# ChristodoulosPappas/IPLS-Java-API

Hardware: AMD Instinct MI355X
Metric: aggregated-gradient GB/s (device-resident), 32 peers×4M doubles/partition (higher is better)
Workload: dtype f64

## Files before the change

ipls-java-api_amd/csrc/ipls_kernels.hpp:

```cpp
#pragma once

#include <hip/hip_runtime.h>
#include <stdint.h>

#ifndef IPLS_ROT
#define IPLS_ROT 0
#endif
#ifndef IPLS_ROUND_PAIRS
#define IPLS_ROUND_PAIRS 1
#endif

namespace ipls {

typedef double d2 __attribute__((ext_vector_type(2)));
typedef unsigned long long u2 __attribute__((ext_vector_type(2)));
typedef unsigned u4w __attribute__((ext_vector_type(4)));

constexpr int kBlock = 256;

enum Start : int { kAccum = 0, kZero = 1, kFirst = 2 };

struct PartDesc {
  int64_t len;
  unsigned long long* dst;
  const unsigned long long* init;
  const unsigned long long* rep;
  unsigned long long* avg;
};

#define IPLS_GLOBAL __attribute__((address_space(1)))
typedef const IPLS_GLOBAL u2* gcu2;
typedef IPLS_GLOBAL u2* gu2;
typedef const IPLS_GLOBAL unsigned long long* gcu64;
typedef IPLS_GLOBAL unsigned long long* gu64;

__device__ __forceinline__ double be_to_f64(unsigned long long v) {
  return __builtin_bit_cast(double, __builtin_bswap64(v));
}
__device__ __forceinline__ unsigned long long f64_to_be(double v) {
  return __builtin_bswap64(__builtin_bit_cast(unsigned long long, v));
}

template <bool NT>
__device__ __forceinline__ u2 ld16(const unsigned long long* p) {
  if constexpr (NT) return __builtin_nontemporal_load((gcu2)p);
  else return *(gcu2)p;
}
__device__ __forceinline__ unsigned long long ld8(const unsigned long long* p) { return *(gcu64)p; }
__device__ __forceinline__ void st8(unsigned long long* p, unsigned long long v) { *(gu64)p = v; }

template <bool BE>
__device__ __forceinline__ d2 decode2(u2 raw) {
  if constexpr (BE) {
    const unsigned long long a = raw.x, b = raw.y;
    u2 s;
    s.x = __builtin_bswap64(a);
    s.y = __builtin_bswap64(b);
    return __builtin_bit_cast(d2, s);
  } else {
    return __builtin_bit_cast(d2, raw);
  }
}
template <bool BE>
__device__ __forceinline__ u2 encode2(d2 v) {
  u2 raw = __builtin_bit_cast(u2, v);
  if constexpr (BE) {
    const unsigned long long a = raw.x, b = raw.y;
    raw.x = __builtin_bswap64(a);
    raw.y = __builtin_bswap64(b);
  }
  return raw;
}
template <bool BE>
__device__ __forceinline__ double decode1(unsigned long long raw) {
  if constexpr (BE) return be_to_f64(raw);
  else return __builtin_bit_cast(double, raw);
}

__host__ __device__ constexpr int64_t grid_blocks(int map, int64_t tiles) {
  return map == 2 ? (tiles + 7) / 8 * 8 : tiles;
}

__device__ __forceinline__ void map_block(int map, int nblocks, int tiles_per_part, int n_parts, int& q, int& t) {
  int b = blockIdx.x;
  if (map == 3) {
    if (b < n_parts) {
      q = b;
      t = tiles_per_part - 1;
    } else {
      b -= n_parts;
      q = b / (tiles_per_part - 1);
      t = b - q * (tiles_per_part - 1);
    }
    return;
  }
  if (map == 2) {
    const int per = nblocks >> 3;
    b = (blockIdx.x & 7) * per + (blockIdx.x >> 3);
    if (b >= tiles_per_part * n_parts) { q = n_parts; t = 0; return; }
  }
  if (map == 1) {
    q = b % n_parts;
    t = b / n_parts;
  } else {
    q = b / tiles_per_part;
    t = b - q * tiles_per_part;
  }
}

template <bool BE_IN, bool BE_OUT, int START, int G, int R, bool NT, int MAP, int BS, bool FIN, int SEQF>
__device__ __forceinline__ void reduce_tiles(
    const unsigned long long* const* __restrict__ bufs, const PartDesc* __restrict__ parts,
    int k, int tiles_per_part, int n_parts, int secure, const double* __restrict__ cnts) {
  constexpr int kBlock = BS;
  constexpr int64_t kTile = (int64_t)kBlock * 2 * R;
  int q, t;
  map_block(MAP, gridDim.x, tiles_per_part, n_parts, q, t);
  if (q >= n_parts) return;
  const int64_t L = parts[q].len;
  const int64_t base = (int64_t)t * kTile;
  if (base >= L) return;
  unsigned long long* __restrict__ dst = parts[q].dst;
  const unsigned long long* const* __restrict__ pb = bufs + (size_t)q * k;
  const int tid = threadIdx.x;
  const int j0 = (START == kFirst) ? 1 : 0;
  static_assert(!(FIN && BE_OUT), "the fused round writes native Weights");
  const unsigned long long* __restrict__ init = FIN ? parts[q].init : dst;
  const unsigned long long* __restrict__ rep = FIN ? parts[q].rep : nullptr;
  unsigned long long* __restrict__ avg = FIN ? parts[q].avg : nullptr;
  double den = 0.0, cnt = 0.0;
  if constexpr (FIN) {
    if (avg) {
      cnt = cnts[q];
      den = secure ? 1e12 * cnt : cnt;
    }
  }
  const bool avg_aligned = FIN && !((uintptr_t)avg & 15);
  auto fin1 = [&](int64_t e, double a) {
    const double w = a + (rep ? __builtin_bit_cast(double, ld8(rep + e)) : 0.0);
    st8(dst + e, __builtin_bit_cast(unsigned long long, w));
    if (avg && e < L - 1) st8(avg + e, __builtin_bit_cast(unsigned long long, cnt == 0.0 ? w : w / den));
  };

  if (base + kTile <= L) {
    int64_t off[R];
#if IPLS_ROT
    const int rot = t & (R - 1);
#else
    constexpr int rot = 0;
#endif
    constexpr bool PAIRS = FIN && IPLS_ROUND_PAIRS && (R % 2 == 0);
    if constexpr (PAIRS) {
#pragma unroll
      for (int r = 0; r < R; ++r)
        off[r] = base + 2 * ((int64_t)(r >> 1) * 2 * kBlock + (tid >> 6) * 128 + (r & 1) * 64 + (tid & 63));
    } else {
#pragma unroll
      for (int r = 0; r < R; ++r) off[r] = base + 2 * ((int64_t)((r + rot) & (R - 1)) * kBlock + tid);
    }

    constexpr bool SEQ = SEQF > 0 && G == 1;
    d2 acc[R];
#pragma unroll
    for (int r = 0; r < R; ++r) {
      if constexpr (START == kZero) {
        acc[r] = d2{0.0, 0.0};
      } else if constexpr (START == kFirst) {
        acc[r] = decode2<BE_IN>(ld16<NT>(pb[0] + off[r]));
      } else {
        acc[r] = decode2<BE_OUT>(ld16<false>(init + off[r]));
      }
      if constexpr (SEQ && START != kZero) __builtin_amdgcn_sched_barrier(0);
    }
    int j = j0;
    if constexpr (SEQ) {
      for (; j < k; ++j) {
        const unsigned long long* __restrict__ src = pb[j];
#pragma unroll
        for (int r = 0; r < R; ++r) {
          const d2 x = decode2<BE_IN>(ld16<NT>(src + off[r]));
          acc[r].x = acc[r].x + x.x;
          acc[r].y = acc[r].y + x.y;
          if constexpr (SEQF > 0)
            if ((r + 1) % (SEQF % 10) == 0 && r + 1 < R - SEQF / 10) __builtin_amdgcn_sched_barrier(0);
        }
      }
    } else {
    for (; j + G <= k; j += G) {
      u2 v[G][R];
#pragma unroll
      for (int g = 0; g < G; ++g) {
        const unsigned long long* __restrict__ src = pb[j + g];
#pragma unroll
        for (int r = 0; r < R; ++r) v[g][r] = ld16<NT>(src + off[r]);
      }
#pragma unroll
      for (int g = 0; g < G; ++g) {
#pragma unroll
        for (int r = 0; r < R; ++r) {
          d2 x = decode2<BE_IN>(v[g][r]);
          acc[r].x = acc[r].x + x.x;
          acc[r].y = acc[r].y + x.y;
        }
      }
    }
    for (; j < k; ++j) {
      const unsigned long long* __restrict__ src = pb[j];
      u2 v[R];
#pragma unroll
      for (int r = 0; r < R; ++r) v[r] = ld16<NT>(src + off[r]);
#pragma unroll
      for (int r = 0; r < R; ++r) {
        d2 x = decode2<BE_IN>(v[r]);
        acc[r].x = acc[r].x + x.x;
        acc[r].y = acc[r].y + x.y;
      }
    }
    }
    if constexpr (FIN) {
#pragma unroll
      for (int r = 0; r < R; ++r) {
        if (rep) {
          const d2 y = decode2<false>(ld16<true>(rep + off[r]));
          acc[r].x = acc[r].x + y.x;
          acc[r].y = acc[r].y + y.y;
        } else {
          acc[r].x = acc[r].x + 0.0;
          acc[r].y = acc[r].y + 0.0;
        }
        if (avg) {
          const int64_t e = off[r];
          const double ax = cnt == 0.0 ? acc[r].x : acc[r].x / den;
          const double ay = cnt == 0.0 ? acc[r].y : acc[r].y / den;
          if (avg_aligned) {
            if (e + 1 < L - 1) __builtin_nontemporal_store(encode2<false>(d2{ax, ay}), (gu2)(avg + e));
            else st8(avg + e, __builtin_bit_cast(unsigned long long, ax));
          } else if constexpr (PAIRS) {
            const int lane = tid & 63;
            const double nx = __shfl_down(ax, 1);
            if ((r & 1) == 0) {
              const double nb = acc[r + 1].x + (rep && lane == 0 ? __builtin_bit_cast(double, ld8(rep + off[r + 1])) : 0.0);
              const double b0 = __shfl(cnt == 0.0 ? nb : nb / den, 0);
              if (lane == 0) st8(avg + e, __builtin_bit_cast(unsigned long long, ax));
              __builtin_nontemporal_store(encode2<false>(d2{ay, lane < 63 ? nx : b0}), (gu2)(avg + e + 1));
            } else {
              if (lane < 63) __builtin_nontemporal_store(encode2<false>(d2{ay, nx}), (gu2)(avg + e + 1));
              else if (e + 1 < L - 1) st8(avg + e + 1, __builtin_bit_cast(unsigned long long, ay));
            }
          } else {
            const double nx = __shfl_down(ax, 1);
            const int lane = tid & 63;
            if (lane == 0) st8(avg + e, __builtin_bit_cast(unsigned long long, ax));
            if (lane < 63) __builtin_nontemporal_store(encode2<false>(d2{ay, nx}), (gu2)(avg + e + 1));
            else if (e + 1 < L - 1) st8(avg + e + 1, __builtin_bit_cast(unsigned long long, ay));
          }
        }
      }
#pragma unroll
      for (int r = 0; r < R; ++r) __builtin_nontemporal_store(encode2<false>(acc[r]), (gu2)(dst + off[r]));
    } else {
#pragma unroll
      for (int r = 0; r < R; ++r) __builtin_nontemporal_store(encode2<BE_OUT>(acc[r]), (gu2)(dst + off[r]));
    }
  } else {
    constexpr int kPB = 8;
    for (int64_t sb = base; sb < L; sb += 2 * kBlock) {
      const int64_t i = sb + 2 * tid;
      if (sb + 2 * kBlock <= L) {
        d2 acc;
        if constexpr (START == kZero) acc = d2{0.0, 0.0};
        else if constexpr (START == kFirst) acc = decode2<BE_IN>(ld16<NT>(pb[0] + i));
        else acc = decode2<BE_OUT>(ld16<false>(init + i));
        int jj = j0;
        for (; jj + kPB <= k; jj += kPB) {
          u2 v[kPB];
#pragma unroll
          for (int g = 0; g < kPB; ++g) v[g] = ld16<NT>(pb[jj + g] + i);
#pragma unroll
          for (int g = 0; g < kPB; ++g) {
            const d2 x = decode2<BE_IN>(v[g]);
            acc.x = acc.x + x.x;
            acc.y = acc.y + x.y;
          }
        }
        for (; jj < k; ++jj) {
          const d2 x = decode2<BE_IN>(ld16<NT>(pb[jj] + i));
          acc.x = acc.x + x.x;
          acc.y = acc.y + x.y;
        }
        if constexpr (FIN) {
          fin1(i, acc.x);
          fin1(i + 1, acc.y);
        } else {
          __builtin_nontemporal_store(encode2<BE_OUT>(acc), (gu2)(dst + i));
        }
      } else {
        for (int64_t e = sb + tid; e < L; e += kBlock) {
          double acc;
          if constexpr (START == kZero) acc = 0.0;
          else if constexpr (START == kFirst) acc = decode1<BE_IN>(ld8(pb[0] + e));
          else acc = decode1<BE_OUT>(ld8(init + e));
          int jj = j0;
          for (; jj + kPB <= k; jj += kPB) {
            unsigned long long v[kPB];
#pragma unroll
            for (int g = 0; g < kPB; ++g) v[g] = ld8(pb[jj + g] + e);
#pragma unroll
            for (int g = 0; g < kPB; ++g) acc = acc + decode1<BE_IN>(v[g]);
          }
          for (; jj < k; ++jj) acc = acc + decode1<BE_IN>(ld8(pb[jj] + e));
          if constexpr (FIN) fin1(e, acc);
          else st8(dst + e, BE_OUT ? f64_to_be(acc) : __builtin_bit_cast(unsigned long long, acc));
        }
      }
    }
  }
}

template <bool BE_IN, bool BE_OUT, int START, int G, int R, bool NT, int MAP = 0, int BS = kBlock, int SEQF = 0>
__global__ __launch_bounds__(BS) void k_reduce(const unsigned long long* const* __restrict__ bufs,
                                               const PartDesc* __restrict__ parts, int k, int tiles_per_part,
                                               int n_parts) {
  reduce_tiles<BE_IN, BE_OUT, START, G, R, NT, MAP, BS, false, SEQF>(bufs, parts, k, tiles_per_part, n_parts, 0,
                                                                     nullptr);
}

template <bool BE_IN, int START, int G, int R, int MAP = 0, int BS = kBlock, int SEQF = 0>
__global__ __launch_bounds__(BS) void k_round(const unsigned long long* const* __restrict__ bufs,
                                              const PartDesc* __restrict__ parts, int k, int tiles_per_part,
                                              int n_parts, int secure, const double* __restrict__ cnts) {
  reduce_tiles<BE_IN, false, START, G, R, true, MAP, BS, true, SEQF>(bufs, parts, k, tiles_per_part, n_parts, secure,
                                                               cnts);
}

constexpr int kEwV = 4;
constexpr int64_t kEwTile = (int64_t)kBlock * 2 * kEwV;

template <bool BE_IN, bool FIRST, bool VEC = false>
__global__ __launch_bounds__(kBlock) void k_fold_n(unsigned long long* __restrict__ dst,
                                                   const unsigned long long* __restrict__ src, int64_t n) {
  auto one = [&](int64_t i) {
    const double x = decode1<BE_IN>(ld8(src + i));
    const double y = FIRST ? x : __builtin_bit_cast(double, ld8(dst + i)) + x;
    st8(dst + i, __builtin_bit_cast(unsigned long long, y));
  };
  if constexpr (VEC) {
    const int64_t base = (int64_t)blockIdx.x * kEwTile;
    if (base + kEwTile <= n) {
      u2 sv[kEwV], dv[kEwV];
#pragma unroll
      for (int v = 0; v < kEwV; ++v) {
        const int64_t i = base + 2 * ((int64_t)v * kBlock + threadIdx.x);
        sv[v] = __builtin_nontemporal_load((gcu2)(src + i));
        if constexpr (!FIRST) dv[v] = *(gcu2)(dst + i);
      }
#pragma unroll
      for (int v = 0; v < kEwV; ++v) {
        const int64_t i = base + 2 * ((int64_t)v * kBlock + threadIdx.x);
        d2 o = decode2<BE_IN>(sv[v]);
        if constexpr (!FIRST) {
          const d2 y = __builtin_bit_cast(d2, dv[v]);
          o.x = y.x + o.x;
          o.y = y.y + o.y;
        }
        *(gu2)(dst + i) = __builtin_bit_cast(u2, o);
      }
      return;
    }
    for (int64_t i = base + threadIdx.x; i < n; i += kBlock) one(i);
  } else {
    for (int64_t i = (int64_t)blockIdx.x * kBlock + threadIdx.x; i < n; i += (int64_t)gridDim.x * kBlock) one(i);
  }
}

template <bool BE_IN, int START>
__global__ __launch_bounds__(64) void k_round_counts(const unsigned long long* const* __restrict__ bufs,
                                                     const PartDesc* __restrict__ parts, int k, int n_parts,
                                                     double* __restrict__ cnts) {
  const int q = blockIdx.x;
  if (q >= n_parts) return;
  const int lane = threadIdx.x;
  const PartDesc d = parts[q];
  const int64_t e = d.len - 1;
  const unsigned long long* const* pb = bufs + (size_t)q * k;
  double c = (START == kZero) ? 0.0 : __builtin_bit_cast(double, ld8(d.init + e));
  for (int j0 = 0; j0 < k; j0 += 64) {
    const int j = j0 + lane;
    const double v = j < k ? decode1<BE_IN>(ld8(pb[j] + e)) : 0.0;
    const int m = k - j0 < 64 ? k - j0 : 64;
    for (int t = 0; t < m; ++t) c = c + __shfl(v, t);
  }
  if (lane == 0) cnts[q] = c + (d.rep ? __builtin_bit_cast(double, ld8(d.rep + e)) : 0.0);
}

template <bool BE_IN, bool BE_OUT, int START>
__global__ __launch_bounds__(kBlock) void k_reduce_scalar(
    const unsigned long long* const* __restrict__ bufs, const PartDesc* __restrict__ parts,
    int k, int tiles_per_part, int64_t tile) {
  const int q = blockIdx.x / tiles_per_part;
  const int t = blockIdx.x - q * tiles_per_part;
  const int64_t L = parts[q].len;
  const int64_t base = (int64_t)t * tile;
  if (base >= L) return;
  unsigned long long* __restrict__ dst = parts[q].dst;
  const unsigned long long* const* __restrict__ pb = bufs + (size_t)q * k;
  const int64_t end = (base + tile < L) ? base + tile : L;
  const int j0 = (START == kFirst) ? 1 : 0;
  for (int64_t i = base + threadIdx.x; i < end; i += kBlock) {
    double acc;
    if constexpr (START == kZero) acc = 0.0;
    else if constexpr (START == kFirst) acc = decode1<BE_IN>(ld8(pb[0] + i));
    else acc = decode1<BE_OUT>(ld8(dst + i));
    for (int j = j0; j < k; ++j) acc = acc + decode1<BE_IN>(ld8(pb[j] + i));
    st8(dst + i, BE_OUT ? f64_to_be(acc) : __builtin_bit_cast(unsigned long long, acc));
  }
}

template <bool BE_IN, bool BE_OUT, int START, int R = 4>
__global__ __launch_bounds__(kBlock) void k_fold1(unsigned long long* __restrict__ dst,
                                                  const unsigned long long* __restrict__ src, int64_t L) {
  const int64_t n2 = L >> 1;
  const int64_t stride = (int64_t)gridDim.x * kBlock * R;
  auto fold = [&](const u2& v, const u2& t) -> u2 {
    const d2 x = decode2<BE_IN>(v);
    if constexpr (START == kFirst) return encode2<BE_OUT>(x);
    d2 a = (START == kZero) ? d2{0.0, 0.0} : decode2<BE_OUT>(t);
    a.x = a.x + x.x;
    a.y = a.y + x.y;
    return encode2<BE_OUT>(a);
  };
  int64_t b = (int64_t)blockIdx.x * kBlock * R + threadIdx.x;
  for (; b + (int64_t)(R - 1) * kBlock < n2; b += stride) {
    u2 v[R], t[R];
#pragma unroll
    for (int r = 0; r < R; ++r) v[r] = ld16<true>(src + 2 * (b + r * kBlock));
    if constexpr (START == kAccum) {
#pragma unroll
      for (int r = 0; r < R; ++r) t[r] = ld16<false>(dst + 2 * (b + r * kBlock));
    }
#pragma unroll
    for (int r = 0; r < R; ++r) __builtin_nontemporal_store(fold(v[r], t[r]), (gu2)(dst + 2 * (b + r * kBlock)));
  }
  for (int r = 0; r < R; ++r) {
    const int64_t i2 = b + r * kBlock;
    if (i2 < n2) {
      const u2 t = (START == kAccum) ? ld16<false>(dst + 2 * i2) : u2{0, 0};
      __builtin_nontemporal_store(fold(ld16<true>(src + 2 * i2), t), (gu2)(dst + 2 * i2));
    }
  }
  if ((L & 1) && blockIdx.x == 0 && threadIdx.x == 0) {
    const int64_t e = L - 1;
    const double x = decode1<BE_IN>(ld8(src + e));
    double a;
    if constexpr (START == kFirst) a = x;
    else a = ((START == kZero) ? 0.0 : decode1<BE_OUT>(ld8(dst + e))) + x;
    st8(dst + e, BE_OUT ? f64_to_be(a) : __builtin_bit_cast(unsigned long long, a));
  }
}

struct FinDesc {
  int64_t len;
  int64_t agg_off, rep_off, w_off;
};

constexpr int kFinV = 8, kDivV = 4;
constexpr int64_t kFinTile = (int64_t)kBlock * 2 * kFinV, kDivTile = (int64_t)kBlock * 2 * kDivV;

template <bool REP_ZERO, bool ZERO_ACC, int BS = kBlock, int V = kFinV>
__global__ __launch_bounds__(BS) void k_finalize(const FinDesc* __restrict__ parts,
                                                 double* __restrict__ arena,
                                                 int tiles_per_part) {
  constexpr int kBlock = BS;
  constexpr int kV = V;
  constexpr int64_t kTile = (int64_t)kBlock * 2 * kV;
  const int q = blockIdx.x / tiles_per_part;
  const int t = blockIdx.x - q * tiles_per_part;
  const FinDesc d = parts[q];
  const int64_t base = (int64_t)t * kTile;
  if (base >= d.len) return;
  const int64_t end = (base + kTile < d.len) ? base + kTile : d.len;
  double* agg = arena + d.agg_off;
  double* rep = arena + d.rep_off;
  double* w = arena + d.w_off;
  if (end - base == kTile) {
    u2 a[kV], r[kV];
#pragma unroll
    for (int v = 0; v < kV; ++v) {
      const int64_t i = base + 2 * ((int64_t)v * kBlock + threadIdx.x);
      a[v] = __builtin_nontemporal_load((gcu2)(agg + i));
      if constexpr (!REP_ZERO) r[v] = __builtin_nontemporal_load((gcu2)(rep + i));
    }
#pragma unroll
    for (int v = 0; v < kV; ++v) {
      const int64_t i = base + 2 * ((int64_t)v * kBlock + threadIdx.x);
      const d2 x = __builtin_bit_cast(d2, a[v]);
      const d2 y = REP_ZERO ? d2{0.0, 0.0} : __builtin_bit_cast(d2, r[v]);
      d2 o;
      o.x = x.x + y.x;
      o.y = x.y + y.y;
      __builtin_nontemporal_store(__builtin_bit_cast(u2, o), (gu2)(w + i));
      if constexpr (ZERO_ACC) {
        __builtin_nontemporal_store(u2{0, 0}, (gu2)(agg + i));
        if constexpr (!REP_ZERO) __builtin_nontemporal_store(u2{0, 0}, (gu2)(rep + i));
      }
    }
    return;
  }
  for (int64_t i = base + threadIdx.x; i < end; i += kBlock) {
    const double a = agg[i];
    const double r = REP_ZERO ? 0.0 : rep[i];
    w[i] = a + r;
    if constexpr (ZERO_ACC) {
      agg[i] = 0.0;
      if constexpr (!REP_ZERO) rep[i] = 0.0;
    }
  }
}

struct DivDesc {
  int64_t len;
  int64_t w_off;
  int64_t out_off;
};

template <bool OUT_BE, bool SECURE, int BS = kBlock, int V = kDivV>
__global__ __launch_bounds__(BS) void k_divide(const DivDesc* __restrict__ parts,
                                               const double* __restrict__ arena,
                                               unsigned long long* __restrict__ out,
                                               int tiles_per_part) {
  constexpr int kBlock = BS;
  constexpr int kV = V;
  constexpr int64_t kTile = (int64_t)kBlock * 2 * kV;
  static_assert(BS % 64 == 0, "whole waves");
  const int q = blockIdx.x / tiles_per_part;
  const int t = blockIdx.x - q * tiles_per_part;
  const DivDesc d = parts[q];
  const int64_t n = d.len - 1;
  const double* w = arena + d.w_off;
  const double cnt = w[d.len - 1];
  const double den = SECURE ? 1e12 * cnt : cnt;
  auto f = [&](double x) -> unsigned long long {
    const double y = (cnt == 0.0) ? x : x / den;
    unsigned long long bits = __builtin_bit_cast(unsigned long long, y);
    if constexpr (OUT_BE) {
      if (y != y) bits = 0x7ff8000000000000ULL;
      bits = __builtin_bswap64(bits);
    }
    return bits;
  };
  unsigned long long* o = out + d.out_off;
  const int64_t to_line = (16 - (int64_t)(((uintptr_t)o >> 3) & 15)) & 15;
  const int64_t head = to_line < n ? to_line : n;
  if (t == 0 && threadIdx.x < head) o[threadIdx.x] = f(w[threadIdx.x]);
  const int64_t base = (int64_t)t * kTile + head;
  if (base >= n) return;
  if (base + kTile <= n) {
    const int64_t wave_base = base + (int64_t)(threadIdx.x >> 6) * 128 * kV + 2 * (threadIdx.x & 63);
    double x[kV][2];
#pragma unroll
    for (int v = 0; v < kV; ++v) {
      const int64_t i = wave_base + (int64_t)v * 128;
      x[v][0] = __builtin_nontemporal_load((const __attribute__((address_space(1))) double*)(w + i));
      x[v][1] = __builtin_nontemporal_load((const __attribute__((address_space(1))) double*)(w + i + 1));
    }
#pragma unroll
    for (int v = 0; v < kV; ++v) {
      const int64_t i = wave_base + (int64_t)v * 128;
      u2 v2;
      v2.x = f(x[v][0]);
      v2.y = f(x[v][1]);
      __builtin_nontemporal_store(v2, (gu2)(o + i));
    }
    return;
  }
  for (int64_t i = base + threadIdx.x; i < n; i += kBlock) o[i] = f(w[i]);
}

template <bool BE_IN, bool BE_OUT, int MODE, bool VEC = false>
__global__ __launch_bounds__(kBlock) void k_split(const unsigned long long* __restrict__ flat,
                                                  int64_t lo, int64_t ncopy, int64_t L,
                                                  unsigned long long* __restrict__ dst) {
  static_assert(MODE == 0 || !BE_OUT, "the folds write native doubles");
  auto one = [&](int64_t i) {
    double v;
    if (i < ncopy) v = decode1<BE_IN>(flat[lo + i]);
    else if (i == ncopy) v = 1.0;
    else v = 0.0;
    if constexpr (MODE == 1) {
      const double a = __builtin_bit_cast(double, dst[i]);
      dst[i] = __builtin_bit_cast(unsigned long long, a + v);
    } else if constexpr (MODE == 2) {
      dst[i] = __builtin_bit_cast(unsigned long long, 0.0 + v);
    } else {
      dst[i] = BE_OUT ? f64_to_be(v) : __builtin_bit_cast(unsigned long long, v);
    }
  };
  if constexpr (VEC) {
    const int64_t base = (int64_t)blockIdx.x * kEwTile;
    if (base + kEwTile <= ncopy) {
      const unsigned long long* src = flat + lo;
      u2 sv[kEwV], dv[kEwV];
#pragma unroll
      for (int k = 0; k < kEwV; ++k) {
        const int64_t i = base + 2 * ((int64_t)k * kBlock + threadIdx.x);
        sv[k] = __builtin_nontemporal_load((gcu2)(src + i));
        if constexpr (MODE == 1) dv[k] = *(gcu2)(dst + i);
      }
#pragma unroll
      for (int k = 0; k < kEwV; ++k) {
        const int64_t i = base + 2 * ((int64_t)k * kBlock + threadIdx.x);
        const d2 x = decode2<BE_IN>(sv[k]);
        d2 o;
        if constexpr (MODE == 1) {
          const d2 a = __builtin_bit_cast(d2, dv[k]);
          o = d2{a.x + x.x, a.y + x.y};
        } else if constexpr (MODE == 2) {
          o = d2{0.0 + x.x, 0.0 + x.y};
        } else {
          o = x;
        }
        *(gu2)(dst + i) = encode2<BE_OUT>(o);
      }
      return;
    }
    const int64_t end = base + kEwTile < L ? base + kEwTile : L;
    for (int64_t i = base + threadIdx.x; i < end; i += kBlock) one(i);
  } else {
    const int64_t i = (int64_t)blockIdx.x * kBlock + threadIdx.x;
    if (i < L) one(i);
  }
}

template <bool VEC = false>
__global__ __launch_bounds__(kBlock) void k_bswap64(const unsigned long long* __restrict__ in,
                                                    unsigned long long* __restrict__ out, int64_t n) {
  if constexpr (VEC) {
    const int64_t base = (int64_t)blockIdx.x * kEwTile;
    if (base + kEwTile <= n) {
      u2 v[kEwV];
#pragma unroll
      for (int k = 0; k < kEwV; ++k) v[k] = __builtin_nontemporal_load((gcu2)(in + base + 2 * ((int64_t)k * kBlock + threadIdx.x)));
#pragma unroll
      for (int k = 0; k < kEwV; ++k) {
        const unsigned long long a = v[k].x, b = v[k].y;
        __builtin_nontemporal_store(u2{__builtin_bswap64(a), __builtin_bswap64(b)},
                                    (gu2)(out + base + 2 * ((int64_t)k * kBlock + threadIdx.x)));
      }
      return;
    }
    for (int64_t i = base + threadIdx.x; i < n; i += kBlock) out[i] = __builtin_bswap64(in[i]);
  } else {
    for (int64_t i = (int64_t)blockIdx.x * kBlock + threadIdx.x; i < n; i += (int64_t)gridDim.x * kBlock)
      out[i] = __builtin_bswap64(in[i]);
  }
}

template <bool BE_IN>
__global__ __launch_bounds__(kBlock) void k_load_model(const unsigned long long* __restrict__ flat,
                                                       int64_t lo, int64_t ncopy, int64_t L,
                                                       double* __restrict__ dst) {
  const int64_t i = (int64_t)blockIdx.x * kBlock + threadIdx.x;
  if (i >= L) return;
  dst[i] = (i < ncopy) ? decode1<BE_IN>(flat[lo + i]) : 0.0;
}

__device__ __forceinline__ unsigned long long splitmix64(unsigned long long v) {
  unsigned long long z = v + 0x9E3779B97F4A7C15ULL;
  z = (z ^ (z >> 30)) * 0xBF58476D1CE4E5B9ULL;
  z = (z ^ (z >> 27)) * 0x94D049BB133111EBULL;
  return z ^ (z >> 31);
}

template <bool BE_OUT>
__global__ __launch_bounds__(kBlock) void k_synth(unsigned long long* __restrict__ dst, int64_t L,
                                                  unsigned long long key) {
  for (int64_t i = (int64_t)blockIdx.x * kBlock + threadIdx.x; i < L;
       i += (int64_t)gridDim.x * kBlock) {
    double x;
    if (i == L - 1) {
      x = 1.0;
    } else {
      const double u = (double)(splitmix64(key ^ (unsigned long long)i) >> 11) * 0x1.0p-53;
      double tt = 2.0 * u;
      tt = tt - 1.0;
      x = tt * 1e-2;
    }
    dst[i] = BE_OUT ? f64_to_be(x) : __builtin_bit_cast(unsigned long long, x);
  }
}

__device__ __forceinline__ unsigned long long dpp_shift(unsigned long long v, int ctrl_id) {
  const int lo = (int)(unsigned)v, hi = (int)(unsigned)(v >> 32);
  int rl, rh;
  switch (ctrl_id) {
    case 0: rl = __builtin_amdgcn_update_dpp(0, lo, 0x111, 0xF, 0xF, true);
            rh = __builtin_amdgcn_update_dpp(0, hi, 0x111, 0xF, 0xF, true); break;
    case 1: rl = __builtin_amdgcn_update_dpp(0, lo, 0x112, 0xF, 0xF, true);
            rh = __builtin_amdgcn_update_dpp(0, hi, 0x112, 0xF, 0xF, true); break;
    case 2: rl = __builtin_amdgcn_update_dpp(0, lo, 0x114, 0xF, 0xF, true);
            rh = __builtin_amdgcn_update_dpp(0, hi, 0x114, 0xF, 0xF, true); break;
    case 3: rl = __builtin_amdgcn_update_dpp(0, lo, 0x118, 0xF, 0xF, true);
            rh = __builtin_amdgcn_update_dpp(0, hi, 0x118, 0xF, 0xF, true); break;
    case 4: rl = __builtin_amdgcn_update_dpp(0, lo, 0x142, 0xA, 0xF, false);
            rh = __builtin_amdgcn_update_dpp(0, hi, 0x142, 0xA, 0xF, false); break;
    default: rl = __builtin_amdgcn_update_dpp(0, lo, 0x143, 0xC, 0xF, false);
             rh = __builtin_amdgcn_update_dpp(0, hi, 0x143, 0xC, 0xF, false); break;
  }
  return ((unsigned long long)(unsigned)rh << 32) | (unsigned)rl;
}

__device__ __forceinline__ unsigned long long wave_sum_u64(unsigned long long v) {
#pragma unroll
  for (int c = 0; c < 6; ++c) v += dpp_shift(v, c);
  const unsigned lo = __builtin_amdgcn_readlane((int)(unsigned)v, 63);
  const unsigned hi = __builtin_amdgcn_readlane((int)(unsigned)(v >> 32), 63);
  return ((unsigned long long)hi << 32) | lo;
}

template <bool BE_IN>
__global__ __launch_bounds__(kBlock) void k_checksum(const unsigned long long* __restrict__ x,
                                                     int64_t n, unsigned long long* __restrict__ out) {
  __shared__ unsigned long long lds[kBlock / 64];
  unsigned long long s = 0;
  for (int64_t i = (int64_t)blockIdx.x * kBlock + threadIdx.x; i < n;
       i += (int64_t)gridDim.x * kBlock) {
    unsigned long long b = BE_IN ? __builtin_bswap64(x[i]) : x[i];
    s += splitmix64(b + (unsigned long long)i * 0x9E3779B97F4A7C15ULL);
  }
  s = wave_sum_u64(s);
  const int lane = threadIdx.x & 63, wid = threadIdx.x >> 6;
  if (lane == 0) lds[wid] = s;
  __syncthreads();
  if (threadIdx.x == 0) {
    unsigned long long t = 0;
#pragma unroll
    for (int w = 0; w < kBlock / 64; ++w) t += lds[w];
    atomicAdd(out, t);
  }
}

struct B64Desc {
  int64_t src_off;
  int64_t units;
  int64_t dst_off;
  int32_t tail;
  int32_t pad;
};

__device__ __forceinline__ unsigned b64url_val(unsigned c) {
  if (c - 'A' < 26u) return c - 'A';
  if (c - 'a' < 26u) return c - 'a' + 26;
  if (c - '0' < 10u) return c - '0' + 52;
  if (c == '-') return 62;
  if (c == '_') return 63;
  return 0x100;
}

__device__ __forceinline__ unsigned b64url_unit(unsigned w) {
  const unsigned a = b64url_val(w & 0xFF), b = b64url_val((w >> 8) & 0xFF);
  const unsigned c = b64url_val((w >> 16) & 0xFF), d = b64url_val(w >> 24);
  return (a << 18) | (b << 12) | (c << 6) | d | ((a | b | c | d) & 0x100 ? 0x1000000u : 0u);
}

__global__ __launch_bounds__(kBlock) void k_b64url_decode(const unsigned char* __restrict__ src,
                                                          const B64Desc* __restrict__ descs,
                                                          unsigned char* __restrict__ dst,
                                                          int* __restrict__ err) {
  const int m = blockIdx.y;
  const B64Desc d = descs[m];
  const unsigned char* s = src + d.src_off;
  unsigned char* o = dst + d.dst_off;
  const int64_t u0 = ((int64_t)blockIdx.x * kBlock + threadIdx.x) * 4;
  if (u0 > d.units) return;
  unsigned bad = 0;
  if (u0 + 4 <= d.units) {
    typedef unsigned u4 __attribute__((ext_vector_type(4)));
    const u4 w = *(const IPLS_GLOBAL u4*)(s + 4 * u0);
    const unsigned v[4] = {b64url_unit(w.x), b64url_unit(w.y), b64url_unit(w.z), b64url_unit(w.w)};
    bad = (v[0] | v[1] | v[2] | v[3]) & 0x1000000u;
    unsigned char* q = o + 3 * u0;
#pragma unroll
    for (int i = 0; i < 4; ++i) {
      q[3 * i] = (unsigned char)(v[i] >> 16);
      q[3 * i + 1] = (unsigned char)(v[i] >> 8);
      q[3 * i + 2] = (unsigned char)v[i];
    }
  } else {
    for (int64_t u = u0; u < d.units; ++u) {
      const unsigned char* c = s + 4 * u;
      const unsigned w = c[0] | (c[1] << 8) | (c[2] << 16) | ((unsigned)c[3] << 24);
      const unsigned v = b64url_unit(w);
      bad |= v & 0x1000000u;
      o[3 * u] = (unsigned char)(v >> 16);
      o[3 * u + 1] = (unsigned char)(v >> 8);
      o[3 * u + 2] = (unsigned char)v;
    }
    if (d.tail && u0 + 4 > d.units) {
      const unsigned char* c = s + 4 * d.units;
      unsigned v = 0, inval = 0;
      for (int i = 0; i < d.tail; ++i) {
        const unsigned x = b64url_val(c[i]);
        inval |= x;
        v |= (x & 63u) << (18 - 6 * i);
      }
      bad |= inval & 0x100;
      o[3 * d.units] = (unsigned char)(v >> 16);
      if (d.tail == 3) o[3 * d.units + 1] = (unsigned char)(v >> 8);
    }
  }
  if (bad) atomicOr(err + m, 1);
}

struct FrameEnc {
  unsigned char hdr[16];
  int64_t n;
  int64_t origin_len;
  const unsigned char* origin;
};

__device__ __forceinline__ unsigned b64url_char(unsigned v) {
  return v < 26 ? 'A' + v : v < 52 ? 'a' + (v - 26) : v < 62 ? '0' + (v - 52) : v == 62 ? '-' : '_';
}
__device__ __forceinline__ unsigned b64url_quad(unsigned v) {
  return b64url_char((v >> 18) & 63) | (b64url_char((v >> 12) & 63) << 8) | (b64url_char((v >> 6) & 63) << 16) |
         (b64url_char(v & 63) << 24);
}

__device__ __forceinline__ unsigned frame_byte(const FrameEnc& f, const unsigned long long* __restrict__ src,
                                               int64_t j) {
  if (j < 14) return f.hdr[j];
  const int64_t q = j - 14;
  if (q < 8 * f.n) {
    if (!src) return 0;
    const unsigned long long v = ld8(src + (q >> 3));
    return (unsigned)(v >> (8 * (7 - (q & 7)))) & 0xFF;
  }
  return f.origin[q - 8 * f.n];
}

__device__ __forceinline__ unsigned b64url_quad_lut(const unsigned char* tab, unsigned v) {
  return (unsigned)tab[(v >> 18) & 63] | ((unsigned)tab[(v >> 12) & 63] << 8) | ((unsigned)tab[(v >> 6) & 63] << 16) |
         ((unsigned)tab[v & 63] << 24);
}

__device__ __forceinline__ void encode_frame_job(const FrameEnc& f, const unsigned long long* __restrict__ src,
                                                 unsigned char* __restrict__ out, int64_t groups, int64_t text_len,
                                                 const unsigned char* tab, u4w* stage) {
  const int lane = threadIdx.x & 63, wv = threadIdx.x >> 6;
  u4w* ws = stage + 128 * wv;
  const int64_t F = 14 + 8 * f.n + f.origin_len;
  for (int64_t g0 = (int64_t)blockIdx.x * kBlock; g0 < groups; g0 += (int64_t)gridDim.x * kBlock) {
    const int64_t gw = g0 + 64 * wv;
    const int64_t g = gw + lane;
    const int64_t b0 = 24 * g;
    u4w c0 = {0u, 0u, 0u, 0u}, c1 = {0u, 0u, 0u, 0u};
    if (g < groups && g >= 1 && b0 + 24 <= 14 + 8 * f.n && src) {
      const unsigned long long* s = src + (3 * g - 2);
      const unsigned long long v0 = ld8(s), v1 = ld8(s + 1), v2 = ld8(s + 2), v3 = ld8(s + 3);
      const unsigned W[8] = {(unsigned)(v0 >> 32), (unsigned)v0, (unsigned)(v1 >> 32), (unsigned)v1,
                             (unsigned)(v2 >> 32), (unsigned)v2, (unsigned)(v3 >> 32), (unsigned)v3};
      unsigned O[6];
#pragma unroll
      for (int k = 0; k < 6; ++k) O[k] = (W[k] << 16) | (W[k + 1] >> 16);
      const unsigned long long X0 = ((unsigned long long)O[0] << 32) | O[1];
      const unsigned long long X1 = ((unsigned long long)O[2] << 32) | O[3];
      const unsigned long long X2 = ((unsigned long long)O[4] << 32) | O[5];
      c0.x = b64url_quad_lut(tab, (unsigned)(X0 >> 40) & 0xFFFFFF);
      c0.y = b64url_quad_lut(tab, (unsigned)(X0 >> 16) & 0xFFFFFF);
      c0.z = b64url_quad_lut(tab, (unsigned)((X0 << 8) | (X1 >> 56)) & 0xFFFFFF);
      c0.w = b64url_quad_lut(tab, (unsigned)(X1 >> 32) & 0xFFFFFF);
      c1.x = b64url_quad_lut(tab, (unsigned)(X1 >> 8) & 0xFFFFFF);
      c1.y = b64url_quad_lut(tab, (unsigned)((X1 << 16) | (X2 >> 48)) & 0xFFFFFF);
      c1.z = b64url_quad_lut(tab, (unsigned)(X2 >> 24) & 0xFFFFFF);
      c1.w = b64url_quad_lut(tab, (unsigned)X2 & 0xFFFFFF);
    } else if (g < groups) {
      unsigned q8[8] = {0u, 0u, 0u, 0u, 0u, 0u, 0u, 0u};
      for (int u = 0; u < 8; ++u) {
        const int64_t j = b0 + 3 * u;
        if (j >= F) break;
        const int nb = F - j >= 3 ? 3 : (int)(F - j);
        unsigned v = frame_byte(f, src, j) << 16;
        if (nb > 1) v |= frame_byte(f, src, j + 1) << 8;
        if (nb > 2) v |= frame_byte(f, src, j + 2);
        unsigned q = b64url_quad(v);
        if (nb < 3) q = (q & 0x00FFFFFFu) | ((unsigned)'=' << 24);
        if (nb < 2) q = (q & 0xFF00FFFFu) | ((unsigned)'=' << 16);
        q8[u] = q;
      }
      c0 = u4w{q8[0], q8[1], q8[2], q8[3]};
      c1 = u4w{q8[4], q8[5], q8[6], q8[7]};
    }
    ws[2 * lane] = c0;
    ws[2 * lane + 1] = c1;
    __builtin_amdgcn_wave_barrier();
    const int64_t wbase = 32 * gw;
#pragma unroll
    for (int h = 0; h < 2; ++h) {
      const u4w v = ws[64 * h + lane];
      const int64_t o = wbase + 1024 * h + 16 * lane;
      if (o + 16 <= text_len) {
        __builtin_nontemporal_store(v, (IPLS_GLOBAL u4w*)(out + o));
      } else if (o < text_len) {
        const unsigned w4[4] = {v.x, v.y, v.z, v.w};
        for (int64_t c = 0; o + c < text_len; ++c) out[o + c] = (unsigned char)(w4[c >> 2] >> (8 * (c & 3)));
      }
    }
    __builtin_amdgcn_wave_barrier();
  }
}

__device__ __forceinline__ void init_b64url_table(unsigned char* tab) {
  if (threadIdx.x < 64) tab[threadIdx.x] = (unsigned char)b64url_char(threadIdx.x);
  __syncthreads();
}

__global__ __launch_bounds__(kBlock) void k_b64url_encode_frame(FrameEnc f, const unsigned long long* __restrict__ src,
                                                               unsigned char* __restrict__ out, int64_t groups,
                                                               int64_t text_len) {
  __shared__ u4w stage[2 * kBlock];
  __shared__ unsigned char tab[64];
  init_b64url_table(tab);
  encode_frame_job(f, src, out, groups, text_len, tab, stage);
}

struct FrameJob {
  FrameEnc f;
  const unsigned long long* src;
  unsigned char* out;
  int64_t groups;
  int64_t text_len;
};

__global__ __launch_bounds__(kBlock) void k_b64url_encode_frames(const FrameJob* __restrict__ jobs) {
  __shared__ u4w stage[2 * kBlock];
  __shared__ unsigned char tab[64];
  init_b64url_table(tab);
  const FrameJob& j = jobs[blockIdx.y];
  encode_frame_job(j.f, j.src, j.out, j.groups, j.text_len, tab, stage);
}

template <bool BE_IN, bool VEC = false>
__global__ __launch_bounds__(kBlock) void k_blend(double* __restrict__ t, const unsigned long long* __restrict__ g,
                                                  int64_t L, double a, double b) {
  auto one = [&](int64_t i) {
    const double x = decode1<BE_IN>(ld8(g + i));
    const double aw = a * t[i];
    const double bg = b * x;
    t[i] = aw + bg;
  };
  if constexpr (VEC) {
    const int64_t base = (int64_t)blockIdx.x * kEwTile;
    if (base + kEwTile <= L) {
      u2 gv[kEwV], tv[kEwV];
#pragma unroll
      for (int v = 0; v < kEwV; ++v) {
        const int64_t i = base + 2 * ((int64_t)v * kBlock + threadIdx.x);
        gv[v] = __builtin_nontemporal_load((gcu2)(g + i));
        tv[v] = *(gcu2)(t + i);
      }
#pragma unroll
      for (int v = 0; v < kEwV; ++v) {
        const int64_t i = base + 2 * ((int64_t)v * kBlock + threadIdx.x);
        const d2 x = decode2<BE_IN>(gv[v]);
        const d2 w = __builtin_bit_cast(d2, tv[v]);
        const double awx = a * w.x, bgx = b * x.x, awy = a * w.y, bgy = b * x.y;
        *(gu2)(t + i) = __builtin_bit_cast(u2, d2{awx + bgx, awy + bgy});
      }
      return;
    }
    for (int64_t i = base + threadIdx.x; i < L; i += kBlock) one(i);
  } else {
    for (int64_t i = (int64_t)blockIdx.x * kBlock + threadIdx.x; i < L; i += (int64_t)gridDim.x * kBlock) one(i);
  }
}

template <bool VEC = false>
__global__ __launch_bounds__(kBlock) void k_scale(double* __restrict__ d, const double* __restrict__ s, int64_t L,
                                                  double c) {
  if constexpr (VEC) {
    const int64_t base = (int64_t)blockIdx.x * kEwTile;
    if (base + kEwTile <= L) {
      u2 sv[kEwV];
#pragma unroll
      for (int v = 0; v < kEwV; ++v)
        sv[v] = __builtin_nontemporal_load((gcu2)(s + base + 2 * ((int64_t)v * kBlock + threadIdx.x)));
#pragma unroll
      for (int v = 0; v < kEwV; ++v) {
        const d2 x = __builtin_bit_cast(d2, sv[v]);
        __builtin_nontemporal_store(__builtin_bit_cast(u2, d2{c * x.x, c * x.y}),
                                    (gu2)(d + base + 2 * ((int64_t)v * kBlock + threadIdx.x)));
      }
      return;
    }
    for (int64_t i = base + threadIdx.x; i < L; i += kBlock) d[i] = c * s[i];
  } else {
    for (int64_t i = (int64_t)blockIdx.x * kBlock + threadIdx.x; i < L; i += (int64_t)gridDim.x * kBlock)
      d[i] = c * s[i];
  }
}

__device__ __forceinline__ double encode_secure1(double x) {
  if (x > 10.0) return 10 * 1e12;
  if (x < -10.0) return -10 * 1e12;
  return x * 1e12;
}

template <bool BE_IN, bool BE_OUT, bool VEC = false>
__global__ __launch_bounds__(kBlock) void k_encode_secure(const unsigned long long* __restrict__ src,
                                                          unsigned long long* __restrict__ dst, int64_t n) {
  auto one = [&](int64_t i) {
    const double y = encode_secure1(decode1<BE_IN>(ld8(src + i)));
    st8(dst + i, BE_OUT ? f64_to_be(y) : __builtin_bit_cast(unsigned long long, y));
  };
  if constexpr (VEC) {
    const int64_t base = (int64_t)blockIdx.x * kEwTile;
    if (base + kEwTile <= n) {
      u2 sv[kEwV];
#pragma unroll
      for (int v = 0; v < kEwV; ++v)
        sv[v] = __builtin_nontemporal_load((gcu2)(src + base + 2 * ((int64_t)v * kBlock + threadIdx.x)));
#pragma unroll
      for (int v = 0; v < kEwV; ++v) {
        const d2 x = decode2<BE_IN>(sv[v]);
        __builtin_nontemporal_store(encode2<BE_OUT>(d2{encode_secure1(x.x), encode_secure1(x.y)}),
                                    (gu2)(dst + base + 2 * ((int64_t)v * kBlock + threadIdx.x)));
      }
      return;
    }
    for (int64_t i = base + threadIdx.x; i < n; i += kBlock) one(i);
  } else {
    for (int64_t i = (int64_t)blockIdx.x * kBlock + threadIdx.x; i < n; i += (int64_t)gridDim.x * kBlock) one(i);
  }
}

constexpr int kSerV = 4;
constexpr int64_t kSerTileWords = (int64_t)kBlock * kSerV;
constexpr int kSerPrefixMax = 192;

struct SerPackJob {
  const unsigned long long* src;
  int64_t n;
  int64_t pos;
  int32_t prefix_len;
  int32_t suffix;
  unsigned char prefix[kSerPrefixMax];
};

__device__ __forceinline__ unsigned long long ser_funnel(unsigned long long hi, unsigned long long lo, int s) {
  return s ? (hi << (8 * s)) | (lo >> (64 - 8 * s)) : hi;
}

__device__ __forceinline__ unsigned ser_pack_byte(const SerPackJob& j, int64_t B, int64_t E, int64_t a) {
  if (a < B) return j.prefix[a - j.pos];
  if (a >= E) return (unsigned)j.suffix;
  if (!j.src) return 0;
  const int64_t q = a - B;
  return (unsigned)(ld8(j.src + (q >> 3)) >> (8 * (7 - (q & 7)))) & 0xFF;
}

__global__ __launch_bounds__(kBlock) void k_ser_pack(const SerPackJob* __restrict__ jobs, unsigned char* __restrict__ img) {
  const SerPackJob& j = jobs[blockIdx.y];
  const int64_t B = j.pos + j.prefix_len, E = B + 8 * j.n;
  const int64_t end = E + (j.suffix >= 0 ? 1 : 0);
  int64_t w0 = (B + 15) >> 4, w1 = E >> 4;
  if (w1 < w0) w1 = w0;
  const int s = (int)((16 * w0 - B) & 7);
  const unsigned long long* src = j.src;
  auto compose = [&](unsigned long long a, unsigned long long b, unsigned long long c) {
    return u2{__builtin_bswap64(ser_funnel(a, b, s)), __builtin_bswap64(ser_funnel(b, c, s))};
  };
  for (int64_t t0 = w0 + (int64_t)blockIdx.x * kSerTileWords; t0 < w1; t0 += (int64_t)gridDim.x * kSerTileWords) {
    if (!src) {
#pragma unroll
      for (int v = 0; v < kSerV; ++v) {
        const int64_t w = t0 + (int64_t)v * kBlock + threadIdx.x;
        if (w < w1) __builtin_nontemporal_store(u2{0, 0}, (gu2)(img + 16 * w));
      }
      continue;
    }
    unsigned long long a[kSerV], b[kSerV], c[kSerV];
#pragma unroll
    for (int v = 0; v < kSerV; ++v) {
      const int64_t w = t0 + (int64_t)v * kBlock + threadIdx.x;
      a[v] = b[v] = c[v] = 0;
      if (w < w1) {
        const int64_t k = (16 * w - B) >> 3;
        a[v] = ld8(src + k);
        b[v] = ld8(src + k + 1);
        if (s) c[v] = ld8(src + k + 2);
      }
    }
#pragma unroll
    for (int v = 0; v < kSerV; ++v) {
      const int64_t w = t0 + (int64_t)v * kBlock + threadIdx.x;
      if (w < w1) __builtin_nontemporal_store(compose(a[v], b[v], c[v]), (gu2)(img + 16 * w));
    }
  }
  if (blockIdx.x == 0) {
    const int64_t head_end = w1 > w0 ? 16 * w0 : end;
    for (int64_t a = j.pos + threadIdx.x; a < head_end; a += kBlock) img[a] = (unsigned char)ser_pack_byte(j, B, E, a);
    if (w1 > w0)
      for (int64_t a = 16 * w1 + threadIdx.x; a < end; a += kBlock) img[a] = (unsigned char)ser_pack_byte(j, B, E, a);
  }
}

constexpr unsigned long long kBoxLead = 0x7371007E0002ull;

__device__ __forceinline__ unsigned long long canon_nan_bits(unsigned long long v) {
  return ((v & 0x7FF0000000000000ull) == 0x7FF0000000000000ull && (v & 0x000FFFFFFFFFFFFFull)) ? 0x7FF8000000000000ull : v;
}

__device__ __forceinline__ unsigned ser_box_byte(const SerPackJob& j, int64_t B, int64_t E, int64_t a) {
  if (a < B + 6) return j.prefix[a - j.pos];
  if (a >= E) return (unsigned)j.suffix;
  const int64_t t = a - B, g = t / 14;
  const int o = (int)(t - 14 * g);
  if (o < 6) return (unsigned)(kBoxLead >> (8 * (5 - o))) & 0xFF;
  const unsigned long long v = j.src ? canon_nan_bits(ld8(j.src + g)) : 0;
  return (unsigned)(v >> (8 * (13 - o))) & 0xFF;
}

__global__ __launch_bounds__(kBlock) void k_ser_pack_boxed(const SerPackJob* __restrict__ jobs,
                                                           unsigned char* __restrict__ img) {
  const SerPackJob& j = jobs[blockIdx.y];
  const int64_t B = j.pos + j.prefix_len - 6, E = B + 14 * j.n;
  const int64_t end = E + (j.suffix >= 0 ? 1 : 0);
  int64_t w0 = (B + 6 + 15) >> 4, w1 = E >> 4;
  if (w1 < w0) w1 = w0;
  const unsigned long long* src = j.src;
  for (int64_t t0 = w0 + (int64_t)blockIdx.x * kSerTileWords; t0 < w1; t0 += (int64_t)gridDim.x * kSerTileWords) {
#pragma unroll
    for (int v = 0; v < kSerV; ++v) {
      const int64_t w = t0 + (int64_t)v * kBlock + threadIdx.x;
      if (w >= w1) continue;
      const int64_t t = 16 * w - B, g = t / 14;
      const int o = (int)(t - 14 * g);
      unsigned long long x = 0, y = 0;
      if (src) {
        x = canon_nan_bits(ld8(src + g));
        if (o > 4) y = canon_nan_bits(ld8(src + g + 1));
      }
      const unsigned long long q0 = (kBoxLead << 16) | (x >> 48), q1 = (x << 16) | (kBoxLead >> 32),
                               q2 = (kBoxLead << 32) | (y >> 32), q3 = (y << 32) | (kBoxLead >> 16);
      const int sh = o & 7;
      const unsigned long long lo = o < 8 ? q0 : q1, mid = o < 8 ? q1 : q2, hi = o < 8 ? q2 : q3;
      __builtin_nontemporal_store(u2{__builtin_bswap64(ser_funnel(lo, mid, sh)), __builtin_bswap64(ser_funnel(mid, hi, sh))},
                                  (gu2)(img + 16 * w));
    }
  }
  if (blockIdx.x == 0) {
    const int64_t head_end = w1 > w0 ? 16 * w0 : end;
    for (int64_t a = j.pos + threadIdx.x; a < head_end; a += kBlock) img[a] = (unsigned char)ser_box_byte(j, B, E, a);
    if (w1 > w0)
      for (int64_t a = 16 * w1 + threadIdx.x; a < end; a += kBlock) img[a] = (unsigned char)ser_box_byte(j, B, E, a);
  }
}

struct SerApplyJob {
  double* dst;
  int64_t n;
  int64_t off;
};

__device__ __forceinline__ unsigned long long ser_load_be(const unsigned char* img, int64_t a) {
  const unsigned long long* w = (const unsigned long long*)(img + (a & ~(int64_t)7));
  const int r = (int)(a & 7);
  const unsigned long long m0 = ld8(w);
  if (!r) return __builtin_bswap64(m0);
  return __builtin_bswap64((m0 >> (8 * r)) | (ld8(w + 1) << (64 - 8 * r)));
}

template <bool BLEND>
__global__ __launch_bounds__(kBlock) void k_ser_apply(const SerApplyJob* __restrict__ jobs,
                                                      const unsigned char* __restrict__ img, double a, double b) {
  const SerApplyJob& j = jobs[blockIdx.y];
  double* dst = j.dst;
  auto put = [&](double t, unsigned long long bits) {
    const double x = __builtin_bit_cast(double, bits);
    if constexpr (BLEND) {
      const double aw = a * t, bg = b * x;
      return aw + bg;
    } else {
      return x;
    }
  };
  const bool vec = (((uintptr_t)dst) & 15) == 0;
  const int64_t pairs = vec ? j.n >> 1 : 0;
  const int r = (int)(j.off & 15), rr = r & 7;
  for (int64_t t0 = (int64_t)blockIdx.x * kSerTileWords; t0 < pairs; t0 += (int64_t)gridDim.x * kSerTileWords) {
    u2 m0[kSerV], m1[kSerV], tv[kSerV];
#pragma unroll
    for (int v = 0; v < kSerV; ++v) {
      const int64_t i = t0 + (int64_t)v * kBlock + threadIdx.x;
      if (i < pairs) {
        const unsigned long long* w = (const unsigned long long*)(img + ((j.off + 16 * i) & ~(int64_t)15));
        m0[v] = __builtin_nontemporal_load((gcu2)w);
        m1[v] = r ? *(gcu2)(w + 2) : u2{0, 0};
        if constexpr (BLEND) tv[v] = *(gcu2)(dst + 2 * i);
      }
    }
#pragma unroll
    for (int v = 0; v < kSerV; ++v) {
      const int64_t i = t0 + (int64_t)v * kBlock + threadIdx.x;
      if (i < pairs) {
        const unsigned long long a0 = m0[v].x, a1 = m0[v].y, a2 = m1[v].x, a3 = m1[v].y;
        const unsigned long long l0 = r < 8 ? a0 : a1, l1 = r < 8 ? a1 : a2, l2 = r < 8 ? a2 : a3;
        const unsigned long long e0 = rr ? (l0 >> (8 * rr)) | (l1 << (64 - 8 * rr)) : l0;
        const unsigned long long e1 = rr ? (l1 >> (8 * rr)) | (l2 << (64 - 8 * rr)) : l1;
        d2 t = d2{0.0, 0.0};
        if constexpr (BLEND) t = __builtin_bit_cast(d2, tv[v]);
        const double ox = put(t.x, __builtin_bswap64(e0)), oy = put(t.y, __builtin_bswap64(e1));
        *(gu2)(dst + 2 * i) = __builtin_bit_cast(u2, d2{ox, oy});
      }
    }
  }
  for (int64_t i = 2 * pairs + (int64_t)blockIdx.x * kBlock + threadIdx.x; i < j.n; i += (int64_t)gridDim.x * kBlock)
    dst[i] = put(BLEND ? dst[i] : 0.0, ser_load_be(img, j.off + 8 * i));
}

__global__ __launch_bounds__(kBlock) void k_ser_unbox(const unsigned char* __restrict__ img, int64_t rec0, int64_t g0,
                                                      int64_t g1, unsigned long long* __restrict__ out,
                                                      unsigned* __restrict__ flag) {
  for (int64_t g = g0 + (int64_t)blockIdx.x * kBlock + threadIdx.x; g < g1; g += (int64_t)gridDim.x * kBlock) {
    const int64_t a = rec0 + 14 * (g - g0);
    if (g >= 1 && (ser_load_be(img, a) >> 16) != kBoxLead) *flag = 1u;
    out[g - g0] = ser_load_be(img, a + 6);
  }
}

}
```

Before: 7032.

## Replace f64 division in fused round epilogue with guarded exact reciprocal multiply

Adds an exact_div helper that turns x/den into a multiply by a precomputed reciprocal plus one FMA correction step. It checks exponent ranges so the result matches IEEE division, and falls back to a true divide otherwise. The fused finalize epilogue makes den wave-uniform, computes the reciprocal once per block, and takes the fast path when the whole wavefront is in range. It also restructures the unaligned average store into paired shuffles and rebuilds the epilogue offsets from one base register to save registers. The aim is to cut the expensive software f64 divide from the memory-bound epilogue, at the cost of extra branching and code complexity.

```diff
diff --git a/ipls-java-api_amd/csrc/exact_div.hpp b/ipls-java-api_amd/csrc/exact_div.hpp
--- /dev/null
+++ b/ipls-java-api_amd/csrc/exact_div.hpp
@@ -0,0 +1,40 @@
+#pragma once
+
+#include <stdint.h>
+
+#if defined(__HIPCC__)
+#include <hip/hip_runtime.h>
+#define IPLS_HD __host__ __device__ __forceinline__
+#else
+#define IPLS_HD inline
+#endif
+
+namespace ipls {
+
+constexpr uint32_t kDenLo = 723, kDenHi = 1323;
+constexpr uint32_t kNumLo = 323, kNumHi = 1723;
+
+IPLS_HD uint32_t f64_hi(double v) { return (uint32_t)(__builtin_bit_cast(uint64_t, v) >> 32); }
+
+IPLS_HD bool exact_div_den_ok(double d) {
+  const uint64_t b = __builtin_bit_cast(uint64_t, d);
+  const uint32_t ex = (uint32_t)(b >> 52) & 0x7ffu;
+  const uint64_t ones = (1ull << 52) - 1;
+  return ex - kDenLo <= kDenHi - kDenLo && (b & ones) != ones;
+}
+
+IPLS_HD bool exact_div_num_ok(double x) { return ((f64_hi(x) >> 20) & 0x7ffu) - kNumLo <= kNumHi - kNumLo; }
+
+IPLS_HD double exact_div_rcp(double x, double d, double y) {
+  const double q0 = x * y;
+  const double e = __builtin_fma(-d, q0, x);
+  return __builtin_fma(e, y, q0);
+}
+
+IPLS_HD double exact_div_guarded(double x, double d, double y, bool den_ok) {
+  return (den_ok && exact_div_num_ok(x)) ? exact_div_rcp(x, d, y) : x / d;
+}
+
+IPLS_HD double exact_div(double x, double d) { return exact_div_guarded(x, d, 1.0 / d, exact_div_den_ok(d)); }
+
+}
diff --git a/ipls-java-api_amd/csrc/ipls_kernels.hpp b/ipls-java-api_amd/csrc/ipls_kernels.hpp
--- a/ipls-java-api_amd/csrc/ipls_kernels.hpp
+++ b/ipls-java-api_amd/csrc/ipls_kernels.hpp
@@ -2,12 +2,20 @@
 
 #include <hip/hip_runtime.h>
 #include <stdint.h>
+
+#include "exact_div.hpp"
 
 #ifndef IPLS_ROT
 #define IPLS_ROT 0
 #endif
 #ifndef IPLS_ROUND_PAIRS
 #define IPLS_ROUND_PAIRS 1
+#endif
+#ifndef IPLS_ROUND_RCP
+#define IPLS_ROUND_RCP 1
+#endif
+#ifndef IPLS_ROUND_PAIR_EPI
+#define IPLS_ROUND_PAIR_EPI 1
 #endif
 
 namespace ipls {
@@ -39,6 +47,13 @@
 }
 __device__ __forceinline__ unsigned long long f64_to_be(double v) {
   return __builtin_bswap64(__builtin_bit_cast(unsigned long long, v));
+}
+
+__device__ __forceinline__ double wave_uniform(double v) {
+  const unsigned long long b = __builtin_bit_cast(unsigned long long, v);
+  const unsigned lo = __builtin_amdgcn_readfirstlane((unsigned)b);
+  const unsigned hi = __builtin_amdgcn_readfirstlane((unsigned)(b >> 32));
+  return __builtin_bit_cast(double, ((unsigned long long)hi << 32) | lo);
 }
 
 template <bool NT>
@@ -114,6 +129,8 @@
     int k, int tiles_per_part, int n_parts, int secure, const double* __restrict__ cnts) {
   constexpr int kBlock = BS;
   constexpr int64_t kTile = (int64_t)kBlock * 2 * R;
+  constexpr bool RCP_DIV = FIN && IPLS_ROUND_RCP && BS != 512;
+  constexpr bool PAIR_EPI_ON = FIN && IPLS_ROUND_PAIR_EPI && BS != 512;
   int q, t;
   map_block(MAP, gridDim.x, tiles_per_part, n_parts, q, t);
   if (q >= n_parts) return;
@@ -133,13 +150,35 @@
     if (avg) {
       cnt = cnts[q];
       den = secure ? 1e12 * cnt : cnt;
+      if constexpr (RCP_DIV) den = wave_uniform(den);
     }
   }
   const bool avg_aligned = FIN && !((uintptr_t)avg & 15);
+  double rcp = 0.0;
+  bool rcp_ok = false;
+  auto rcp_setup = [&]() {
+    if constexpr (FIN && RCP_DIV) {
+      if (avg && cnt != 0.0 && exact_div_den_ok(den)) {
+        rcp_ok = true;
+        rcp = 1.0 / den;
+      }
+    }
+  };
+  auto avg1 = [&](double w) -> double {
+    if constexpr (RCP_DIV) return cnt == 0.0 ? w : exact_div_guarded(w, den, rcp, rcp_ok);
+    else return cnt == 0.0 ? w : w / den;
+  };
+  auto avg2 = [&](d2 w) -> d2 {
+    if constexpr (RCP_DIV) {
+      if (rcp_ok && !__any(!(exact_div_num_ok(w.x) && exact_div_num_ok(w.y))))
+        return d2{exact_div_rcp(w.x, den, rcp), exact_div_rcp(w.y, den, rcp)};
+    }
+    return d2{cnt == 0.0 ? w.x : w.x / den, cnt == 0.0 ? w.y : w.y / den};
+  };
   auto fin1 = [&](int64_t e, double a) {
     const double w = a + (rep ? __builtin_bit_cast(double, ld8(rep + e)) : 0.0);
     st8(dst + e, __builtin_bit_cast(unsigned long long, w));
-    if (avg && e < L - 1) st8(avg + e, __builtin_bit_cast(unsigned long long, cnt == 0.0 ? w : w / den));
+    if (avg && e < L - 1) st8(avg + e, __builtin_bit_cast(unsigned long long, avg1(w)));
   };
 
   if (base + kTile <= L) {
@@ -218,36 +257,73 @@
     }
     }
     if constexpr (FIN) {
+      constexpr bool EPI_OFFS = !IPLS_ROT && (RCP_DIV || (PAIRS && PAIR_EPI_ON));
+      int64_t eo[R];
+      if constexpr (EPI_OFFS) {
+        int64_t o0 = off[0];
+        asm volatile("" : "+v"(o0));
+#pragma unroll
+        for (int r = 0; r < R; ++r)
+          eo[r] = o0 + (PAIRS ? 2 * ((int64_t)(r >> 1) * 2 * kBlock + (r & 1) * 64) : 2 * (int64_t)r * kBlock);
+      } else {
+#pragma unroll
+        for (int r = 0; r < R; ++r) eo[r] = off[r];
+      }
+      constexpr bool PAIR_EPI = PAIRS && PAIR_EPI_ON;
+      rcp_setup();
+      auto add_rep = [&](d2& a, int64_t o) {
+        if (rep) {
+          const d2 y = decode2<false>(ld16<true>(rep + o));
+          a.x = a.x + y.x;
+          a.y = a.y + y.y;
+        } else {
+          a.x = a.x + 0.0;
+          a.y = a.y + 0.0;
+        }
+      };
+      const bool by_pairs = PAIR_EPI && avg && !avg_aligned;
 #pragma unroll
       for (int r = 0; r < R; ++r) {
-        if (rep) {
-          const d2 y = decode2<false>(ld16<true>(rep + off[r]));
-          acc[r].x = acc[r].x + y.x;
-          acc[r].y = acc[r].y + y.y;
-        } else {
-          acc[r].x = acc[r].x + 0.0;
-          acc[r].y = acc[r].y + 0.0;
-        }
+        if (!(by_pairs && (r & 1))) add_rep(acc[r], eo[r]);
+        if constexpr (PAIR_EPI)
+          if (by_pairs && !(r & 1)) add_rep(acc[r + 1], eo[r + 1]);
         if (avg) {
-          const int64_t e = off[r];
-          const double ax = cnt == 0.0 ? acc[r].x : acc[r].x / den;
-          const double ay = cnt == 0.0 ? acc[r].y : acc[r].y / den;
+          const int64_t e = eo[r];
+          if constexpr (PAIR_EPI) {
+            if (by_pairs) {
+              if ((r & 1) == 0) {
+                const int lane = tid & 63;
+                const int64_t e1 = eo[r + 1];
+                const d2 a0 = avg2(acc[r]), a1 = avg2(acc[r + 1]);
+                const double a0x = a0.x, a0y = a0.y, a1x = a1.x, a1y = a1.y;
+                const double nx0 = __shfl_down(a0x, 1), nx1 = __shfl_down(a1x, 1);
+                const double b0 = __shfl(a1x, 0);
+                if (lane == 0) st8(avg + e, __builtin_bit_cast(unsigned long long, a0x));
+                __builtin_nontemporal_store(encode2<false>(d2{a0y, lane < 63 ? nx0 : b0}), (gu2)(avg + e + 1));
+                if (lane < 63) __builtin_nontemporal_store(encode2<false>(d2{a1y, nx1}), (gu2)(avg + e1 + 1));
+                else if (e1 + 1 < L - 1) st8(avg + e1 + 1, __builtin_bit_cast(unsigned long long, a1y));
+              }
+              continue;
+            }
+          }
+          const d2 a = avg2(acc[r]);
+          const double ax = a.x, ay = a.y;
           if (avg_aligned) {
             if (e + 1 < L - 1) __builtin_nontemporal_store(encode2<false>(d2{ax, ay}), (gu2)(avg + e));
             else st8(avg + e, __builtin_bit_cast(unsigned long long, ax));
-          } else if constexpr (PAIRS) {
+          } else if constexpr (PAIRS && !PAIR_EPI) {
             const int lane = tid & 63;
             const double nx = __shfl_down(ax, 1);
             if ((r & 1) == 0) {
-              const double nb = acc[r + 1].x + (rep && lane == 0 ? __builtin_bit_cast(double, ld8(rep + off[r + 1])) : 0.0);
-              const double b0 = __shfl(cnt == 0.0 ? nb : nb / den, 0);
+              const double nb = acc[r + 1].x + (rep && lane == 0 ? __builtin_bit_cast(double, ld8(rep + eo[r + 1])) : 0.0);
+              const double b0 = __shfl(avg1(nb), 0);
               if (lane == 0) st8(avg + e, __builtin_bit_cast(unsigned long long, ax));
               __builtin_nontemporal_store(encode2<false>(d2{ay, lane < 63 ? nx : b0}), (gu2)(avg + e + 1));
             } else {
               if (lane < 63) __builtin_nontemporal_store(encode2<false>(d2{ay, nx}), (gu2)(avg + e + 1));
               else if (e + 1 < L - 1) st8(avg + e + 1, __builtin_bit_cast(unsigned long long, ay));
             }
-          } else {
+          } else if constexpr (!PAIRS) {
             const double nx = __shfl_down(ax, 1);
             const int lane = tid & 63;
             if (lane == 0) st8(avg + e, __builtin_bit_cast(unsigned long long, ax));
@@ -257,13 +333,14 @@
         }
       }
 #pragma unroll
-      for (int r = 0; r < R; ++r) __builtin_nontemporal_store(encode2<false>(acc[r]), (gu2)(dst + off[r]));
+      for (int r = 0; r < R; ++r) __builtin_nontemporal_store(encode2<false>(acc[r]), (gu2)(dst + eo[r]));
     } else {
 #pragma unroll
       for (int r = 0; r < R; ++r) __builtin_nontemporal_store(encode2<BE_OUT>(acc[r]), (gu2)(dst + off[r]));
     }
   } else {
     constexpr int kPB = 8;
+    rcp_setup();
     for (int64_t sb = base; sb < L; sb += 2 * kBlock) {
       const int64_t i = sb + 2 * tid;
       if (sb + 2 * kBlock <= L) {
```

After: 7034, median of 6. No clear change (+0.0%).
